# csyxwei/FFWM

Measured on AMD Instinct MI355X. Metric: train img/s (128x128, full FFWM GAN step), higher is better.
Workload: dtype f32; 1 GPU; BASELINE configs[2]: full FFWM train step (netG+netD+flowNetF+flowNetB, all losses, 3x Adam), synthetic MultiPIE-shaped 128x128; batch_per_gpu=8, global_batch=8, parallelism=dp1, grad_buckets=10, bucket_MiB=64

## Files before the change

### ffwm_amd/_lib.py

```python
import ctypes
import os

_HERE = os.path.dirname(os.path.abspath(__file__))
LIB_PATH = os.path.join(_HERE, "lib", "libffwm_hip.so")

F32, F64 = 0, 1
ABI_VERSION = 5

_lib = None

_p = ctypes.c_void_p
_i64 = ctypes.c_int64
_i = ctypes.c_int

_SIGNATURES = {
    "ffwm_block_extractor_forward": [_p, _p, _p] + [_i64] * 6 + [_i, _i, _p],
    "ffwm_block_extractor_backward": [_p, _p, _p, _p, _p] + [_i64] * 6 + [_i, _i, _p],
    "ffwm_block_extractor_backward_strided": [_p, _p, _p, ctypes.POINTER(_i64), _p, _p] + [_i64] * 6 + [_i, _i, _p],
    "ffwm_local_attn_reshape_backward_strided": [_p, ctypes.POINTER(_i64), _p] + [_i64] * 3 + [_i, _i, _i, _p],
    "ffwm_resample2d_backward_strided": [_p, _p, _p, ctypes.POINTER(_i64), _p, _p] + [_i64] * 6 + [_i, _i, _i, _i, _p],
    "ffwm_bn_lrelu_forward": [_p] * 9 + [_i64] * 3 + [ctypes.c_double] * 3 + [_i, _p],
    "ffwm_bn_lrelu_backward": [_p] * 10 + [_i64] * 3 + [ctypes.c_double] + [_i, _p],
    "ffwm_bn_res_act_forward": [_p] * 11 + [_i64] * 3 + [ctypes.c_double] * 3 + [_i, _i, _p],
    "ffwm_bn_res_act_backward": [_p] * 11 + [_i64] * 3 + [ctypes.c_double] + [_i, _i, _p],
# ... 3 lines not shown
    "ffwm_add_act_backward": [_p, _p, _p, _i64, _i, ctypes.c_double, _i, _p],
    "ffwm_sigmoid_gate_forward": [_p, _p, _p, _p, _p, _i64, _i, _p],
    "ffwm_sigmoid_gate_backward": [_p, _p, _p, _p, _p, _i64, _i, _p],
    "ffwm_bias_relu_forward": [_p, _p, _p] + [_i64] * 3 + [_i, _p],
    "ffwm_bias_act_forward": [_p, _p, _p, _p] + [_i64] * 5 + [_i, ctypes.c_double, _i, _p],
    "ffwm_flow_head_forward": [_p, _p, _p, _p] + [_i64] * 4 + [_i, _p],
    "ffwm_conv_thin_forward": [_p, _p, _p, _p] + [_i64] * 5 + [_i, ctypes.c_double, _i, _p],
    "ffwm_flow_up_forward": [_p, _p, _p, _p] + [_i64] * 4 + [_i, _p],
    "ffwm_shuffle_bias_act_forward": [_p, _p, _p] + [_i64] * 5 + [ctypes.c_double, _i, _p],
    "ffwm_image_head_forward": [_p, _p, _p, _p] + [_i64] * 5 + [_i, _p],
    "ffwm_upsample2x_bilinear_forward": [_p, _p] + [_i64] * 5 + [_i, _p],
    "ffwm_sigmoid_gate_forward_strided": [_p, _p, _p, _p, _p] + [_i64] * 4 + [_i, _p],
    "ffwm_flow_head_backward": [_p, _p, _p, _p, _p] + [_i64] * 4 + [_i, _p],
    "ffwm_flow_up_backward": [_p, _p, _p] + [_i64] * 4 + [_i, _p],
    "ffwm_conv2d_forward": [_p, _p, _p, _p, _p] + [_i64] * 5 + [_i, _i, _i, _i, _i64, _i64, _i, ctypes.c_double, _p, _i64, _i, _p],
    "ffwm_conv2d_wgrad": [_p, _p, _p] + [_i64] * 7 + [_i, _i, _i, _i, _p],
    "ffwm_conv2d_wgrad_tiled": [_p, _p, _p, _p] + [_i64] * 7 + [_i, _i, _i, _i, _i, _p],
    "ffwm_conv3x3_winograd_forward": [_p, _p, _p, _p, _p] + [_i64] * 5 + [_i, _i, ctypes.c_double, _i, _p],
    "ffwm_adam_step": [_p, _p, _p, _p, _i64] + [ctypes.c_double] * 4 + [_i64, _i, _p],
    "ffwm_adam_step_device": [_p, _p, _p, _p, _i64] + [ctypes.c_double] * 4 + [_p, _i, _p],
    "ffwm_sgd_step": [_p, _p, _p, _i64, _p, _p, _i, _p, _p, _i, ctypes.c_double, _i, _p],
    "ffwm_softmax_xent": [_p] * 8 + [_i64, _i64, _i, _p],
    "ffwm_softmax_xent_chunk": [],
    "ffwm_conv3x3_wgrad": [_p, _p, _p, _p] + [_i64] * 5 + [_i, _p],
    "ffwm_conv3x3_wgrad_block": [_p, _p, _p, _p] + [_i64] * 9 + [_i, _p],
    "ffwm_block_attention_forward": [_p, _p, _p, _p] + [_i64] * 6 + [_i, _i, _p],
    "ffwm_block_attention_backward": [_p, _p, _p, _p, _p, _p, _p] + [_i64] * 6 + [_i, _i, _p],
    "ffwm_local_attn_reshape_forward": [_p, _p] + [_i64] * 3 + [_i, _i, _p],
    "ffwm_local_attn_reshape_backward": [_p, _p] + [_i64] * 3 + [_i, _i, _i, _p],
    "ffwm_resample2d_forward": [_p, _p, _p] + [_i64] * 6 + [_i, _i, _i, _p],
    "ffwm_resample2d_backward": [_p, _p, _p, _p, _p] + [_i64] * 6 + [_i, _i, _i, _i, _p],
    "ffwm_warp_forward": [_p, _p, _p] + [_i64] * 6 + [_i, _i, _p],
    "ffwm_warp_backward": [_p, _p, _p, _p, _p] + [_i64] * 6 + [_i, _i, _p],
    "ffwm_warp_multi_forward": [_p, _i, _i, _i, _p],
    "ffwm_warp_multi_backward": [_p, _i, _i, _i, _p],
    "ffwm_spectral_norm_forward": [_p, _i, _i, ctypes.c_double, _i, _p],
    "ffwm_spectral_norm_backward": [_p, _i, _i, _p],
    "ffwm_guided_filter_forward": [_p, _p, _p, _p, _i64, _i64, _i64, _i, ctypes.c_double, _i, _p],
    "ffwm_affine_regularization": [_p, _p, _p, _p, _i64, _i64, _i64, _i, ctypes.c_double, _i, _p],
    "ffwm_correlation_colmax": [_p, _p, _p, _i64, _i64, _i64, _i, _p],
    "ffwm_correlation_colmax_split": [_p, _p, _p, _i64, _i64, _i64, _i, _p],
    "ffwm_sampling_correctness": [_p] * 9 + [_i64] * 6 + [ctypes.c_double, ctypes.c_double, _i, _p],
    "ffwm_landmark_loss": [_p, _p, ctypes.POINTER(_i64), ctypes.POINTER(_i64), ctypes.POINTER(ctypes.c_double), _i] + [_p] * 6
                          + [_i64, _i64, _i, _p],
    "ffwm_guided_filter_backward": [_p, _p, _p, _p, _p, _p, _i64, _i64, _i64, _i, _i, _p],
    "ffwm_guided_filter_forward_general": [_p, _p, _p, _p, _p, _i64, _i64, _i64, _i64, _i, ctypes.c_double, _i, _p],
    "ffwm_guided_filter_backward_general": [_p, _p, _p, _p, _p, _p, _p, _i64, _i64, _i64, _i64, _i, _i, _p],
    "ffwm_l1_multi": [_p, _i, _p, _p, _i, _i, _p],
    "ffwm_conv3x3_winograd_weights_multi": [_p, _i, _i, _p],
    "ffwm_conv3x3_wg_weights": [_p, _p, _i64, _i64, _i, _i, _p],
    "ffwm_conv3x3_wg_forward": [_p, _p, _p, _p, _p] + [_i64] * 5 + [_i, _p, _i, _p],
    "ffwm_conv3x3_wg_forward_tiled": [_p, _p, _p, _p, _p] + [_i64] * 5 + [_i, _p, _i, _i, _p],
    "ffwm_conv3x3_wg_tile": [_i64] * 5,
    "ffwm_mfm_tail_forward": [_p, _p, _p, _p] + [_i64] * 4 + [_i, _i, _p],
    "ffwm_identity_input": [_p, _p] + [_i64] * 4 + [_i, _i, _p],
    "ffwm_identity_input_backward": [_p, _p] + [_i64] * 4 + [_i, _i, _p],
    "ffwm_cosine_topk": [_p, _p, _p, _p] + [_i64] * 4 + [_p, _i64, _i, _p],
    "ffwm_prof_enable": [_i],
    "ffwm_prof_collect": [],
    "ffwm_prof_get": [_i, ctypes.c_char_p, _i, ctypes.POINTER(_i64), ctypes.POINTER(ctypes.c_double),
                      ctypes.POINTER(ctypes.c_double)],
    "ffwm_prof_get_flops": [_i, ctypes.POINTER(ctypes.c_double)],
    "ffwm_prof_get_bound": [_i, ctypes.POINTER(ctypes.c_double)],
    "ffwm_prof_reset": [],
    "ffwm_set_option": [ctypes.c_char_p, _i],
    "ffwm_zero_fill": [_p, _i64, _p],
    "ffwm_abi_version": [],
}

EXPORTS = sorted(list(_SIGNATURES) + ["ffwm_last_error", "ffwm_conv3x3_winograd_workspace_bytes", "ffwm_conv3x3_winograd_splits",
                                      "ffwm_conv2d_forward_workspace", "ffwm_guided_filter_workspace_bytes",
                                      "ffwm_sampling_correctness_workspace_bytes", "ffwm_landmark_loss_workspace_bytes",
                                      "ffwm_cosine_topk_workspace_bytes", "ffwm_softmax_xent_workspace_bytes",
                                      "ffwm_conv3x3_wg_weights_bytes", "ffwm_conv3x3_wg_workspace_bytes"])


class FFWMError(RuntimeError):
    pass


def load():
    global _lib
    if _lib is not None:
        return _lib
    if not os.path.exists(LIB_PATH):
        raise FFWMError(
            "libffwm_hip.so is missing (%s). The HIP extension is the only implementation of the "
            "ffwm_amd ops -- build it with `python -m ffwm_amd.build`." % LIB_PATH)
    lib = ctypes.CDLL(LIB_PATH)
    for name, argtypes in _SIGNATURES.items():
        fn = getattr(lib, name)
        fn.argtypes = argtypes
        fn.restype = _i
    lib.ffwm_conv3x3_winograd_workspace_bytes.argtypes = [_i64, _i64]
    lib.ffwm_conv3x3_winograd_workspace_bytes.restype = _i64
    lib.ffwm_conv3x3_winograd_splits.argtypes = [_i64, _i64, _i64, _i64, _i64, _i]
    lib.ffwm_conv3x3_winograd_splits.restype = _i
    lib.ffwm_conv2d_forward_workspace.argtypes = [_i64] * 5 + [_i] * 4
    lib.ffwm_conv2d_forward_workspace.restype = _i64
    lib.ffwm_guided_filter_workspace_bytes.argtypes = [_i64] * 4 + [_i, _i]
    lib.ffwm_guided_filter_workspace_bytes.restype = _i64
    lib.ffwm_sampling_correctness_workspace_bytes.argtypes = [_i64, _i64, _i64, _i]
    lib.ffwm_sampling_correctness_workspace_bytes.restype = _i64
    lib.ffwm_landmark_loss_workspace_bytes.argtypes = [ctypes.POINTER(_i64), _i, _i64, _i64, _i]
    lib.ffwm_landmark_loss_workspace_bytes.restype = _i64
    lib.ffwm_softmax_xent_workspace_bytes.argtypes = [_i64, _i64, _i]
# ... 62 lines not shown
```

### ffwm_amd/conv.py

```python
import os as _os

import torch
import torch.nn as nn
from torch.autograd import Function

from . import ops

_WGRAD_W64 = _os.environ.get("FFWM_WGRAD_W64", "1") == "1"


class _Conv3x3MfmaWgrad(Function):

    @staticmethod
    def forward(ctx, x, weight, bias):
        ctx.save_for_backward(x, weight)
        ctx.has_bias = bias is not None
        return torch.ops.aten.convolution(x, weight, bias, [1, 1], [1, 1], [1, 1], False, [0, 0], 1)

    @staticmethod
    @torch.autograd.function.once_differentiable
    def backward(ctx, grad_output):
        x, weight = ctx.saved_tensors
        go = grad_output.contiguous()
        need_x, need_w, need_b = ctx.needs_input_grad[0], ctx.needs_input_grad[1], ctx.has_bias and ctx.needs_input_grad[2]
# ... 373 lines not shown
        if ctx.own_dgrad:
            return ops.conv3x3_wg(go, ctx.entry[1], None, "none", relu_mask=y, K=ctx.C), None, None, None, None
        if ctx.relu:
            go = torch.ops.aten.threshold_backward(go, y, 0)
        gx = torch.ops.aten.convolution_backward(go, x, weight, None, [1, 1], [1, 1], [1, 1], False, [0, 0], 1, [True, False, False])[0]
        return gx, None, None, None, None


def wg_bias_relu(x, layer):
    entry = wg_entry(layer, layer.weight)
    if torch.is_grad_enabled() and x.requires_grad:
        return _WgConv3x3.apply(x, layer.weight, layer.bias, entry, True)
    return ops.conv3x3_wg(x.contiguous(), entry[0], layer.bias, "relu")


def wg_conv(x, layer):
    entry = wg_entry(layer, layer.weight)
    if torch.is_grad_enabled() and x.requires_grad:
        return _WgConv3x3.apply(x, layer.weight, None, entry, False)
    return ops.conv3x3_wg(x.contiguous(), entry[0], None, "none", K=layer.weight.shape[0])


def wg_bias_mfm(x, layer):
    entry = wg_entry(layer, layer.weight)
    return ops.conv3x3_wg(x.contiguous(), entry[0], layer.bias, "mfm", K=layer.weight.shape[0])


def wg_prepare(net):
    n = 0
    if not _WG:
        return n
    for m in net.modules():
        if (isinstance(m, nn.Conv2d) and m.kernel_size == (3, 3) and m.stride == (1, 1) and m.padding == (1, 1) and m.dilation == (1, 1)
                and m.groups == 1 and m.weight.is_cuda and m.weight.dtype == torch.float32 and _wg_class(m.weight)[0] != _WG_NEVER):
            d = wg_entry(m, m.weight)
            if d is not None:
                n += 4 * sum(u.numel() for k, u in d.items() if k != "key")
    return n


def _conv_fwd_call(x, weight, bias, stride, pad, transposed):
    from .flownet_eval import conv_mfma, NONE
    return conv_mfma(x, weight, bias, stride, pad, transposed, NONE)


def _bias_grad(go):
    return go.sum((0, 2, 3))


_OWN_DGRAD = _os.environ.get("FFWM_CONV_DGRAD", "0") == "1"
_OWN_DGRAD_T = _os.environ.get("FFWM_CONVT_DGRAD", "1") != "0"


class _MfmaConv2d(Function):

    @staticmethod
    def forward(ctx, x, weight, bias, stride, pad, own_fwd=True):
        x, weight = x.contiguous(), weight.contiguous()
        ctx.save_for_backward(x, weight)
        ctx.cfg = (stride, pad, bias is not None)
        if own_fwd:
            return _conv_fwd_call(x, weight, bias, stride, pad, False)
        return torch.ops.aten.convolution(x, weight, bias, [stride, stride], [pad, pad], [1, 1], False, [0, 0], 1)

    @staticmethod
    @torch.autograd.function.once_differentiable
    def backward(ctx, grad_output):
        x, weight = ctx.saved_tensors
        stride, pad, has_bias = ctx.cfg
        go = grad_output.contiguous()
        need_x, need_w, need_b = ctx.needs_input_grad[0], ctx.needs_input_grad[1], has_bias and ctx.needs_input_grad[2]
        gx = gw = gb = None
        k = weight.size(2)
        even = x.size(2) == 2 * go.size(2) and x.size(3) == 2 * go.size(3)
        if need_x and _OWN_DGRAD and stride == 2 and pad == 1 and even and min(weight.shape[0], weight.shape[1]) >= 32:
            gx = _conv_fwd_call(go, weight, None, 2, 1, 1 if k == 4 else 2)
            need_x = False
        elif (need_x and k == 3 and stride == 1 and pad == 1 and min(weight.shape[0], weight.shape[1]) >= 32
              and (_OWN_DGRAD or x.size(2) * x.size(3) <= 64)):
            gx = _conv_fwd_call(go, weight, None, 1, 1, 3)
            need_x = False
        if need_w:
            gw, gb = conv_weight_grad(x, go, weight, stride, pad, need_b)
        if need_x:
            gx = torch.ops.aten.convolution_backward(go, x, weight, None, [stride, stride], [pad, pad], [1, 1], False, [0, 0], 1,
                                                     [True, False, False])[0]
        if need_b and gb is None:
            gb = _bias_grad(go)
        return gx, gw, gb, None, None, None


class _MfmaConvTranspose2d(Function):

    @staticmethod
    def forward(ctx, x, weight, bias, own_fwd=True):
        x, weight = x.contiguous(), weight.contiguous()
        ctx.save_for_backward(x, weight)
        ctx.has_bias = bias is not None
        if own_fwd:
            return _conv_fwd_call(x, weight, bias, 2, 1, True)
        return torch.ops.aten.convolution(x, weight, bias, [2, 2], [1, 1], [1, 1], True, [0, 0], 1)

    @staticmethod
    @torch.autograd.function.once_differentiable
    def backward(ctx, grad_output):
        x, weight = ctx.saved_tensors
        go = grad_output.contiguous()
        need_x, need_w, need_b = ctx.needs_input_grad[0], ctx.needs_input_grad[1], ctx.has_bias and ctx.needs_input_grad[2]
        gx = gw = gb = None
        if need_x and _OWN_DGRAD_T and min(weight.shape[0], weight.shape[1]) >= 16:
            gx = _conv_fwd_call(go, weight, None, 2, 1, False)
            need_x = False
        if need_w:
            gw, gb = conv_transpose_weight_grad(x, go, weight, need_b)
        if need_x:
            gx = torch.ops.aten.convolution_backward(go, x, weight, None, [2, 2], [1, 1], [1, 1], True, [0, 0], 1, [True, False, False])[0]
        if need_b and gb is None:
            gb = _bias_grad(go)
        return gx, gw, gb, None


def fwd_route_ok(x, weight):
    return (x.is_cuda and x.dtype == torch.float32 and weight.dtype == torch.float32 and x.dim() == 4 and not torch.is_autocast_enabled()
            and x.numel() < (1 << 29) and weight.numel() < (1 << 29))


class MfmaFwdConv2d(nn.Conv2d):

    def _conv_forward(self, input, weight, bias):
        if fwd_route_ok(input, weight) and (self.stride[0] == 2 or input.size(2) <= 32):
            return _MfmaConv2d.apply(input, weight, bias, self.stride[0], self.padding[0])
        return super()._conv_forward(input, weight, bias)

# ... 192 lines not shown
```

### ffwm_amd/nets.py

```python
import math
import os

import torch
import torch.nn as nn
import torch.nn.functional as F
from torch.nn.utils import spectral_norm

from . import _ext
from . import conv as _conv
from .external_function import WarpFlipCat, WarpNet, warp_many

LRELU = 0.2


def _msra(mods):
    for m in mods:
        if isinstance(m, (nn.Conv2d, nn.ConvTranspose2d)):
            nn.init.kaiming_normal_(m.weight)
            if m.bias is not None:
                nn.init.constant_(m.bias, 0)


def _cbl(cin, cout, stride=1):
    return nn.Sequential(nn.Conv2d(cin, cout, 3, stride, 1, bias=True), nn.BatchNorm2d(cout),
# ... 45 lines not shown
        f = self.conv0(x)
        skips = {}
        for L in range(1, 7):
            f = getattr(self, "conv%d_1" % L)(getattr(self, "conv%d" % L)(f))
            skips[L] = f
        flow = self.predict_flow6(f)
        flows = {}
        cat = None
        for L in range(5, -1, -1):
            up = getattr(self, "upsampled_flow%d_to_%d" % (L + 1, L))(flow)
            d = getattr(self, "deconv%d" % L)(f if L == 5 else cat)
            cat = torch.cat((skips[L], d, up) if L >= 3 else (d, up), 1)
            flow = getattr(self, "predict_flow%d" % L)(getattr(self, "inter_conv%d" % L)(cat))
            flows[L] = flow
        return flows[0], flows[1], flows[2]


class Tanh2(nn.Module):
    def forward(self, x):
        return (torch.tanh(x) + 1) / 2


def _activ(name):
    table = {"relu": nn.ReLU, "lrelu": lambda: nn.LeakyReLU(LRELU), "sigmoid": nn.Sigmoid, "tanh": nn.Tanh,
             "tanh2": Tanh2}
    if name not in table:
        raise NotImplementedError("Activation %s not implemented" % name)
    return table[name]()


def _sn(m, on):
    return spectral_norm(m) if on else m


class ResidualBlock(nn.Module):

    def __init__(self, inc, outc=None, kernel=3, activ="lrelu", sn=True):
        super().__init__()
        outc = inc if outc is None else outc
        pad = kernel // 2 if sn else kernel
        self.activ = _activ(activ)
        self.input = _sn(nn.Conv2d(inc, outc, 1, 1, 0), sn)
        self.blocks = nn.Sequential(_sn(nn.Conv2d(inc, outc, kernel, 1, pad), sn), nn.BatchNorm2d(outc),
                                    nn.LeakyReLU(LRELU), _sn(nn.Conv2d(outc, outc, kernel, 1, pad), sn),
                                    nn.BatchNorm2d(outc))

    def forward(self, x):
        return self.activ(self.blocks(x) + self.input(x))


class FusedResidualBlock(ResidualBlock):

    def forward(self, x):
        from .norm import RES_ACTS, bn_res_act, bn_res_act_ok
        from .residual import _act_of, add_act
        blocks, inp = self.blocks, self.input
        bn = blocks[-1] if isinstance(blocks, nn.Sequential) and len(blocks) >= 2 else None
        act, slope = _act_of(self.activ)
        if (bn is not None and isinstance(inp, nn.Conv2d) and not inp._forward_pre_hooks and not inp._forward_hooks
                and bn_res_act_ok(bn, x, RES_ACTS.get(act)) and torch.is_grad_enabled()):
            h = x
            for m in list(blocks)[:-1]:
                h = m(h)
            s = inp._conv_forward(x, inp.weight, None)
            if h.shape == s.shape and h.shape[1] == bn.num_features:
                return bn_res_act(h, bn, s, inp.bias, RES_ACTS[act], slope)
            return add_act(bn(h), s if inp.bias is None else s + inp.bias.view(1, -1, 1, 1), self.activ)
        return add_act(blocks(x), inp(x), self.activ)


def _conv_block(inc, outc, ks, s, p, activ="lrelu", res=0, bn=True, sn=True):
    layers = [_sn(nn.Conv2d(inc, outc, ks, s, p), sn)]
    if bn:
        layers.append(nn.BatchNorm2d(outc))
    if activ is not None:
        layers.append(_activ(activ))
    layers += [ResidualBlock(outc, activ=activ, sn=sn) for _ in range(res)]
    return nn.Sequential(*layers)


def _shuffle_block(inc, outc, sn=True):
    return nn.Sequential(_sn(nn.Conv2d(inc, outc * 4, 3, 1, 1), sn), nn.PixelShuffle(2), nn.BatchNorm2d(outc),
                         _activ("lrelu"))


class FFWM(nn.Module):

    def __init__(self, num_layers=3, isflip=True, sn=True, warp_flipcat=None):
        super().__init__()
        ch = [64, 64, 128, 256]
        dch = [256, 128, 64, 64]
        self.isflip = isflip
        dm = 3 if isflip else 2
        am = dm - 1
        self.layers = num_layers
        self.e0 = _conv_block(3, ch[0], 7, 1, 3, res=1, bn=False, sn=sn)
        for i in (1, 2, 3):
            setattr(self, "e%d" % i, _conv_block(ch[i - 1], ch[i], 4, 2, 1, res=1, sn=sn))
        d_in = [dch[0], dch[1] * dm, dch[2] * dm + 3]
        r_ch = [dch[1] * dm, dch[2] * dm + 3, dch[3] * dm + 3]
        for i in range(3):
            setattr(self, "d%d" % i, _shuffle_block(d_in[i], dch[i + 1], sn=sn))
        for i in range(3):
            setattr(self, "dres%d" % i, nn.Sequential(*[ResidualBlock(r_ch[i], activ="lrelu", sn=sn) for _ in range(2)]))
        for i in range(3):
            setattr(self, "rec%d" % i, _conv_block(r_ch[i], 3, 3, 1, 1, bn=False, activ="sigmoid", sn=sn))
        for i, c in enumerate((ch[2] * am, ch[1] * am, ch[0] * am)):
            setattr(self, "att%d" % i, nn.Sequential(_conv_block(c, c, 3, 1, 1, sn=sn),
                                                     ResidualBlock(c, c, activ="sigmoid", sn=sn)))
        self.warpNet = WarpNet()
        self._fused = warp_flipcat if warp_flipcat is not None else WarpFlipCat()
        self._multi = warp_flipcat is None and os.environ.get("FFWM_WARP_MULTI", "1") != "0"
        self.fuse_gate = False

    def _skip(self, feat, flow):
        if self.isflip:
            return self._fused(feat, flow)
# ... 263 lines not shown
```

### ffwm_amd/ops.py

```python
import ctypes

import torch

from . import _lib

_DT = {torch.float32: _lib.F32, torch.float64: _lib.F64}


def _dtype_code(t):
    try:
        return _DT[t.dtype]
    except KeyError:
        raise TypeError("ffwm_amd ops support float32/float64 (AT_DISPATCH_FLOATING_TYPES), got %s" % t.dtype)


def _go_strides(grad_output):
    if grad_output.is_contiguous():
        return grad_output, None
    st = grad_output.stride()
    if any(x < 0 for x in st) or st[3] == 0:
        return grad_output.contiguous(), None
    return grad_output, (ctypes.c_int64 * 4)(*st)


# ... 739 lines not shown

WG_EPILOGUES = {"none": 0, "bias": 1, "relu": 2, "mfm": 3}


def conv3x3_wg_weights(weight, data_gradient=False):
    if not (weight.is_cuda and weight.dtype == torch.float32 and weight.is_contiguous() and weight.dim() == 4 and tuple(weight.shape[2:]) == (3, 3)):
        raise ValueError("conv3x3_wg_weights: a contiguous float32 [K, C, 3, 3] weight on the GPU")
    K, C = (weight.shape[1], weight.shape[0]) if data_gradient else (weight.shape[0], weight.shape[1])
    lib = _lib.load()
    U = weight.new_empty((lib.ffwm_conv3x3_wg_weights_bytes(K, C) // 4,))
    with _on_device(weight) as stream:
        _lib.check(lib.ffwm_conv3x3_wg_weights(_ptr(weight), _ptr(U), K, C, int(bool(data_gradient)), _lib.F32, stream), "ffwm_conv3x3_wg_weights")
    return U


def conv3x3_wg(x, U, bias, epilogue, relu_mask=None, out=None, K=None, tile=0):
    _check("conv3x3_wg", x, relu_mask, out)
    for t in (U, bias):
        if t is not None and (t.device != x.device or t.dtype != x.dtype or not t.is_contiguous()):
            raise ValueError("conv3x3_wg: U and bias must be contiguous tensors of the input's device and dtype")
    if x.dtype != torch.float32:
        raise TypeError("conv3x3_wg: float32 only")
    B, C, H, W = x.shape
    if K is None:
        if bias is None:
            raise ValueError("conv3x3_wg: K is needed when there is no bias")
        K = bias.numel()
    lib = _lib.load()
    if U.numel() * 4 != lib.ffwm_conv3x3_wg_weights_bytes(K, C):
        raise ValueError("conv3x3_wg: U does not belong to a layer with %d input and %d output channels" % (C, K))
    if bias is not None and (not bias.is_contiguous() or bias.numel() != K):
        raise ValueError("conv3x3_wg: bias must be a contiguous vector of %d elements" % K)
    if relu_mask is not None and (relu_mask.shape != x.shape or not relu_mask.is_contiguous()):
        raise ValueError("conv3x3_wg: relu_mask must be contiguous and of x's shape")
    epi = WG_EPILOGUES[epilogue]
    if epi == 3 and K % 2:
        raise ValueError("conv3x3_wg: the mfm epilogue needs an even K")
    shape = (B, K // 2 if epi == 3 else K, H, W)
    if out is None:
        out = x.new_empty(shape)
    elif tuple(out.shape) != shape:
        raise ValueError("conv3x3_wg: out has the wrong shape")
    ws = x.new_empty((lib.ffwm_conv3x3_wg_workspace_bytes(B, C, H, W, K) // 4,))
    with _on_device(x) as stream:
        _lib.check(lib.ffwm_conv3x3_wg_forward_tiled(_ptr(x), _ptr(U), _ptr(bias), _ptr(out), _ptr(ws), B, C, H, W, K, epi,
                                                     _ptr(relu_mask), int(tile), _dtype_code(x), stream), "ffwm_conv3x3_wg_forward")
    return out


def conv3x3_wg_tile(B, C, H, W, K):
    return int(_lib.load().ffwm_conv3x3_wg_tile(int(B), int(C), int(H), int(W), int(K)))


def _mfm_dims(x):
    if x.dim() < 2 or x.shape[1] % 2:
        raise ValueError("mfm: need [B, 2C, ...], got %s" % (tuple(x.shape),))
    hw = 1
    for d in x.shape[2:]:
        hw *= d
    return x.shape[0], x.shape[1] // 2, hw


def _bias_ok(x, bias, n):
    if bias is None:
        return
    if not (bias.is_cuda and bias.dtype == x.dtype and bias.is_contiguous() and bias.numel() == n):
        raise ValueError("bias must be a contiguous float32 GPU vector of %d elements" % n)


_ACT_CODES = {"lrelu": 1, "sigmoid": 3}


def _same_f32(name, *ts):
    t0 = ts[0]
    for t in ts:
        if not (t.is_cuda and t.dtype == torch.float32 and t.is_contiguous() and t.shape == t0.shape and t.device == t0.device):
            raise NotImplementedError("%s: contiguous float32 GPU tensors of one shape only" % name)


def add_act_forward(a, b, act, negative_slope=0.2):
    _same_f32("add_act_forward", a, b)
    y = torch.empty_like(a)
    if y.numel():
        with _on_device(a) as stream:
            _lib.check(_lib.load().ffwm_add_act_forward(_ptr(a), _ptr(b), _ptr(y), a.numel(), _ACT_CODES[act], float(negative_slope),
                                                        _lib.F32, stream), "ffwm_add_act_forward")
    return y


def add_act_backward(y, grad_y, act, negative_slope=0.2):
    _same_f32("add_act_backward", y, grad_y)
    dz = torch.empty_like(y)
    if dz.numel():
        with _on_device(y) as stream:
            _lib.check(_lib.load().ffwm_add_act_backward(_ptr(y), _ptr(grad_y), _ptr(dz), y.numel(), _ACT_CODES[act],
                                                         float(negative_slope), _lib.F32, stream), "ffwm_add_act_backward")
    return dz


def sigmoid_gate_forward(a, b, x):
    _same_f32("sigmoid_gate_forward", a, b, x)
    att, y = torch.empty_like(a), torch.empty_like(a)
    if y.numel():
        with _on_device(a) as stream:
            _lib.check(_lib.load().ffwm_sigmoid_gate_forward(_ptr(a), _ptr(b), _ptr(x), _ptr(att), _ptr(y), a.numel(), _lib.F32, stream),
                       "ffwm_sigmoid_gate_forward")
# ... 257 lines not shown
```

### ffwm_amd/residual.py

```python
import torch
import torch.nn as nn
from torch.autograd import Function
from torch.autograd.function import once_differentiable

from . import ops


class _AddAct(Function):
    @staticmethod
    def forward(ctx, a, b, act, slope):
        y = ops.add_act_forward(a.contiguous(), b.contiguous(), act, slope)
        ctx.save_for_backward(y)
        ctx.act, ctx.slope = act, slope
        return y

    @staticmethod
    @once_differentiable
    def backward(ctx, g):
        (y,) = ctx.saved_tensors
        dz = ops.add_act_backward(y, _grad_in(g), ctx.act, ctx.slope)
        return dz, dz, None, None


class _SigmoidGate(Function):
    @staticmethod
    def forward(ctx, a, b, x):
        x = x.contiguous()
        y, att = ops.sigmoid_gate_forward(a.contiguous(), b.contiguous(), x)
        ctx.save_for_backward(x, att)
        ctx.mark_non_differentiable(att)
        return y, att

    @staticmethod
    @once_differentiable
    def backward(ctx, gy, _gatt):
        x, att = ctx.saved_tensors
        dz, dx = ops.sigmoid_gate_backward(x, att, _grad_in(gy))
        return dz, dz, dx


def _act_of(module):
    if isinstance(module, nn.LeakyReLU) and module.negative_slope > 0:
        return "lrelu", float(module.negative_slope)
    if isinstance(module, nn.Sigmoid):
        return "sigmoid", 0.0
    return None, 0.0


def _aligned(t):
    return not t.is_contiguous() or t.data_ptr() % 16 == 0


def _kernel_ok(*ts):
    t0 = ts[0]
    return (t0.is_cuda and not torch.is_autocast_enabled()
            and all(t.dtype == torch.float32 and t.shape == t0.shape and t.device == t0.device and _aligned(t) for t in ts))


def _grad_in(g):
    g = g.contiguous()
    return g if g.data_ptr() % 16 == 0 else g.clone()


def add_act(a, b, activ):
    act, slope = _act_of(activ)
    if act is not None and _kernel_ok(a, b):
        return _AddAct.apply(a, b, act, slope)
    return activ(a + b)


def gated(att_module, skip, fuse=True):
    rb = att_module[-1] if isinstance(att_module, nn.Sequential) and len(att_module) >= 2 else None
    if (fuse and rb is not None and hasattr(rb, "blocks") and hasattr(rb, "input") and isinstance(getattr(rb, "activ", None), nn.Sigmoid)
            and _kernel_ok(skip)):
        h = skip
        for m in list(att_module)[:-1]:
            h = m(h)
        a, b = rb.blocks(h), rb.input(h)
        if _kernel_ok(a, b, skip):
            return _SigmoidGate.apply(a, b, skip)
        att = rb.activ(a + b)
        return skip * att, att
    att = att_module(skip)
    return skip * att, att


def fuse_residual(net):
    from .nets import FusedResidualBlock, ResidualBlock
    n = 0
    for m in net.modules():
        if type(m) is ResidualBlock and _act_of(m.activ)[0] is not None:
            m.__class__ = FusedResidualBlock
            n += 1
    if hasattr(net, "fuse_gate"):
        net.fuse_gate = True
    return n
```

### include/ffwm_hip.h

```cpp
#ifndef FFWM_HIP_H_
#define FFWM_HIP_H_

#include <stdint.h>

#ifdef __cplusplus
extern "C" {
#endif

#define FFWM_ABI_VERSION 5

typedef enum {
    FFWM_OK = 0,
    FFWM_ERR_ARG = -1,
    FFWM_ERR_DTYPE = -2,
    FFWM_ERR_SIZE = -3,
    FFWM_ERR_LAUNCH = -4
} ffwm_status;

typedef enum { FFWM_F32 = 0, FFWM_F64 = 1 } ffwm_dtype;

int ffwm_abi_version(void);
const char* ffwm_last_error(void);

int ffwm_block_extractor_forward(const void* source, const void* flow_field, void* output,
// ... 187 lines not shown
                           int64_t K, int act, double negative_slope, int dtype, void* stream);

int ffwm_flow_head_forward(const void* x, const void* weight, const void* bias, void* y, int64_t B, int64_t C, int64_t H,
                           int64_t W, int dtype, void* stream);
int ffwm_flow_up_forward(const void* flow, const void* weight, const void* bias, void* out, int64_t B, int64_t H, int64_t W,
                         int64_t out_batch_stride, int dtype, void* stream);

int ffwm_flow_head_backward(const void* y, const void* grad_y, const void* weight, void* grad_z, void* grad_x, int64_t B, int64_t C,
                            int64_t H, int64_t W, int dtype, void* stream);
int ffwm_flow_up_backward(const void* grad_out, const void* weight, void* grad_x, int64_t B, int64_t H, int64_t W,
                          int64_t grad_out_batch_stride, int dtype, void* stream);

int64_t ffwm_conv2d_forward_workspace(int64_t B, int64_t C, int64_t H, int64_t W, int64_t K, int kernel, int stride, int pad,
                                      int transposed);
int ffwm_conv2d_forward(const void* input, const void* weight, const void* bias, void* output, void* output2, int64_t B, int64_t C,
                        int64_t H, int64_t W, int64_t K, int kernel, int stride, int pad, int transposed, int64_t out_batch_stride,
                        int64_t out2_batch_stride, int act, double negative_slope, void* workspace, int64_t workspace_bytes,
                        int dtype, void* stream);

int ffwm_conv2d_wgrad(const void* rows, const void* gathered, void* grad_weight, int64_t B, int64_t K, int64_t Ho, int64_t Wo,
                      int64_t C, int64_t H, int64_t W, int kernel, int stride, int pad, int dtype, void* stream);

int ffwm_conv2d_wgrad_tiled(const void* rows, const void* gathered, void* grad_weight, void* grad_bias, int64_t B, int64_t K,
                            int64_t Ho, int64_t Wo, int64_t C, int64_t H, int64_t W, int kernel, int stride, int pad, int prezeroed,
                            int dtype, void* stream);

int64_t ffwm_conv3x3_winograd_workspace_bytes(int64_t K, int64_t C);
int ffwm_conv3x3_winograd_splits(int64_t B, int64_t C, int64_t H, int64_t W, int64_t K, int act);

typedef struct ffwm_wino_weights {
    const void* weight;
    void* workspace;
    int64_t K, C;
    int data_gradient;
    int width_multiple_of_4;
} ffwm_wino_weights;
int ffwm_conv3x3_winograd_weights_multi(const ffwm_wino_weights* items, int n, int dtype, void* stream);
int ffwm_conv3x3_winograd_forward(const void* input, const void* weight, const void* bias, void* output, void* workspace,
                                  int64_t B, int64_t C, int64_t H, int64_t W, int64_t K, int data_gradient, int act,
                                  double slope, int dtype, void* stream);

enum { FFWM_WG_NONE = 0, FFWM_WG_BIAS = 1, FFWM_WG_BIAS_RELU = 2, FFWM_WG_BIAS_MFM = 3 };
int64_t ffwm_conv3x3_wg_weights_bytes(int64_t K, int64_t C);
int64_t ffwm_conv3x3_wg_workspace_bytes(int64_t B, int64_t C, int64_t H, int64_t W, int64_t K);
int ffwm_conv3x3_wg_weights(const void* weight, void* U, int64_t K, int64_t C, int data_gradient, int dtype, void* stream);
int ffwm_conv3x3_wg_forward(const void* input, const void* U, const void* bias, void* output, void* workspace,
                            int64_t B, int64_t C, int64_t H, int64_t W, int64_t K, int epilogue, const void* relu_mask,
                            int dtype, void* stream);
int ffwm_conv3x3_wg_tile(int64_t B, int64_t C, int64_t H, int64_t W, int64_t K);
int ffwm_conv3x3_wg_forward_tiled(const void* input, const void* U, const void* bias, void* output, void* workspace,
                                  int64_t B, int64_t C, int64_t H, int64_t W, int64_t K, int epilogue, const void* relu_mask,
                                  int tile, int dtype, void* stream);

int ffwm_adam_step(void* params, const void* grads, void* exp_avg, void* exp_avg_sq, int64_t n, double lr,
                   double beta1, double beta2, double eps, int64_t step, int dtype, void* stream);

int ffwm_adam_step_device(void* params, const void* grads, void* exp_avg, void* exp_avg_sq, int64_t n, double lr, double beta1,
                          double beta2, double eps, void* state, int dtype, void* stream);

int ffwm_sgd_step(void* params, const void* grads, void* momentum_buf, int64_t n, const int64_t* seg_end, const int32_t* seg_group,
                  int n_seg, const double* group_lr, const double* group_wd, int n_groups, double momentum, int dtype, void* stream);

int ffwm_softmax_xent_chunk(void);
int64_t ffwm_softmax_xent_workspace_bytes(int64_t B, int64_t N, int dtype);
int ffwm_softmax_xent(const void* logits, const int64_t* target, void* out, void* row_loss, int* rank, void* grad_logits,
                      int* skipped, void* workspace, int64_t B, int64_t N, int dtype, void* stream);

int ffwm_shuffle_bias_act_forward(const void* h, const void* bias, void* y, int64_t B, int64_t K, int64_t H, int64_t W,
                                  int64_t y_batch_stride, double negative_slope, int dtype, void* stream);
int ffwm_image_head_forward(const void* x, const void* weight, const void* bias, void* y, int64_t B, int64_t C, int64_t H, int64_t W,
                            int64_t y_batch_stride, int dtype, void* stream);
int ffwm_upsample2x_bilinear_forward(const void* x, void* y, int64_t B, int64_t C, int64_t H, int64_t W, int64_t y_batch_stride,
                                     int dtype, void* stream);
int ffwm_sigmoid_gate_forward_strided(const void* a, const void* b, const void* x, void* att, void* y, int64_t B, int64_t C,
                                      int64_t HW, int64_t y_batch_stride, int dtype, void* stream);

int ffwm_mfm_tail_forward(const void* h, const void* bias, const void* residual, void* y, int64_t B, int64_t C, int64_t H, int64_t W,
                          int pool, int dtype, void* stream);
int ffwm_identity_input(const void* img, void* out, int64_t B, int64_t Cin, int64_t H, int64_t W, int crop, int dtype, void* stream);
int ffwm_identity_input_backward(const void* grad_out, void* grad_img, int64_t B, int64_t Cin, int64_t H, int64_t W, int crop, int dtype,
                                 void* stream);
int64_t ffwm_cosine_topk_workspace_bytes(int64_t B, int64_t G, int64_t D, int64_t k);
int ffwm_cosine_topk(const void* probe, const void* gallery, void* values, void* indices, int64_t B, int64_t G, int64_t D, int64_t k,
                     void* workspace, int64_t workspace_bytes, int dtype, void* stream);

int ffwm_prof_enable(int on);
int ffwm_prof_collect(void);
int ffwm_prof_get(int row, char* name, int name_len, int64_t* launches, double* total_ms,
                  double* algorithmic_bytes);
int ffwm_prof_get_flops(int row, double* algorithmic_flops);
int ffwm_prof_get_bound(int row, double* roofline_ms);
int ffwm_prof_reset(void);

int ffwm_set_option(const char* key, int value);

int ffwm_zero_fill(void* p, int64_t bytes, void* stream);

#ifdef __cplusplus
}
#endif
#endif
```

Baseline: 219.9 img/s.

## Add MFMA 1x1 conv kernel with fused residual dgrad for shortcut convs

Adds a HIP kernel for 1x1 convolutions that uses fp32 MFMA (32x32x2) with double-buffered LDS weight staging and an optional residual add in the epilogue. A shape/pixel-count table decides per layer whether forward and data-gradient go through this kernel or through aten. A new autograd function forks the residual-block shortcut so the shortcut-conv data gradient is fused with the main-branch gradient accumulation, saving a separate add. The aim is to reduce the cost of library 1x1 convs and gradient sums, at the price of a hand-tuned table and more custom-kernel code.

```diff
diff --git a/ffwm_amd/_lib.py b/ffwm_amd/_lib.py
--- a/ffwm_amd/_lib.py
+++ b/ffwm_amd/_lib.py
@@ -79,6 +79,7 @@
     "ffwm_conv3x3_wg_forward": [_p, _p, _p, _p, _p] + [_i64] * 5 + [_i, _p, _i, _p],
     "ffwm_conv3x3_wg_forward_tiled": [_p, _p, _p, _p, _p] + [_i64] * 5 + [_i, _p, _i, _i, _p],
     "ffwm_conv3x3_wg_tile": [_i64] * 5,
+    "ffwm_conv1x1_forward": [_p, _p, _p, _p] + [_i64] * 5 + [_i, _i, _p],
     "ffwm_mfm_tail_forward": [_p, _p, _p, _p] + [_i64] * 4 + [_i, _i, _p],
     "ffwm_identity_input": [_p, _p] + [_i64] * 4 + [_i, _i, _p],
     "ffwm_identity_input_backward": [_p, _p] + [_i64] * 4 + [_i, _i, _p],
diff --git a/ffwm_amd/conv.py b/ffwm_amd/conv.py
--- a/ffwm_amd/conv.py
+++ b/ffwm_amd/conv.py
@@ -449,6 +449,82 @@
 _OWN_DGRAD_T = _os.environ.get("FFWM_CONVT_DGRAD", "1") != "0"
 
 
+_CONV1X1 = _os.environ.get("FFWM_CONV1X1", "1") != "0"
+_C1_NEVER = (1, 0)
+CONV1X1_TABLE = {
+    (64, 64): ((32768, 131072), (32768, 131072)),
+    (128, 128): ((32768, 32768), (8192, 131072)),
+    (195, 195): ((32768, 131072), (32768, 131072)),
+    (256, 256): (_C1_NEVER, (2048, 2048)),
+    (384, 384): (_C1_NEVER, _C1_NEVER),
+}
+CONV1X1_UNLISTED = (_C1_NEVER, _C1_NEVER)
+
+
+def _conv1x1_layer_ok(x, weight):
+    return (_CONV1X1 and weight.dim() == 4 and weight.shape[2] == 1 and weight.shape[3] == 1 and x.dim() == 4
+            and weight.shape[1] == x.shape[1] and min(weight.shape[0], weight.shape[1]) >= 32 and not torch.is_autocast_enabled()
+            and ops.conv1x1_ok(x, weight))
+
+
+def conv1x1_dirs(x, weight):
+    if not _conv1x1_layer_ok(x, weight):
+        return False, False
+    pixels = x.shape[0] * x.shape[2] * x.shape[3]
+    fwd, dgrad = CONV1X1_TABLE.get((weight.shape[1], weight.shape[0]), CONV1X1_UNLISTED)
+    return fwd[0] <= pixels <= fwd[1], dgrad[0] <= pixels <= dgrad[1]
+
+
+def _conv1x1_dgrad(go, x, weight, own, join=None):
+    if own and ops.conv1x1_ok(go, weight, join):
+        return ops.conv1x1(go, weight, transposed=True, residual=join)
+    gx = torch.ops.aten.convolution_backward(go, x, weight, None, [1, 1], [0, 0], [1, 1], False, [0, 0], 1, [True, False, False])[0]
+    return gx if join is None else join + gx
+
+
+class _ShortcutFork(Function):
+
+    @staticmethod
+    def forward(ctx, x, weight, bias, dirs):
+        ctx.set_materialize_grads(False)
+        ctx.save_for_backward(x, weight)
+        ctx.has_bias, ctx.own_dgrad = bias is not None, dirs[1]
+        if dirs[0]:
+            s = ops.conv1x1(x, weight)
+            if bias is not None:
+                s += bias.view(1, -1, 1, 1)
+        else:
+            s = torch.ops.aten.convolution(x, weight, bias, [1, 1], [0, 0], [1, 1], False, [0, 0], 1)
+        return x, s
+
+    @staticmethod
+    @torch.autograd.function.once_differentiable
+    def backward(ctx, g_main, g_s):
+        x, weight = ctx.saved_tensors
+        need_x, need_w, need_b = ctx.needs_input_grad[0], ctx.needs_input_grad[1], ctx.has_bias and ctx.needs_input_grad[2]
+        if g_s is None:
+            return (g_main if need_x else None), None, None, None
+        go = g_s.contiguous()
+        gx = gw = gb = None
+        if need_x:
+            gx = _conv1x1_dgrad(go, x, weight, ctx.own_dgrad, None if g_main is None else g_main.contiguous())
+        if need_w:
+            gw, gb = conv_weight_grad(x, go, weight, 1, 0, need_b)
+        if need_b and gb is None:
+            gb = _bias_grad(go)
+        return gx, gw, gb, None
+
+
+def shortcut_fork(layer, x, with_bias):
+    if (type(layer) is OwnBwdConv2d and layer.kernel_size == (1, 1) and layer.stride == (1, 1) and layer.padding == (0, 0)
+            and not layer._forward_pre_hooks and not layer._forward_hooks
+            and torch.is_grad_enabled() and layer.weight.requires_grad and x.requires_grad and x.is_contiguous()):
+        dirs = conv1x1_dirs(x, layer.weight)
+        if dirs[0] or dirs[1]:
+            return _ShortcutFork.apply(x, layer.weight, layer.bias if with_bias else None, dirs)
+    return x, (layer(x) if with_bias else layer._conv_forward(x, layer.weight, None))
+
+
 class _MfmaConv2d(Function):
 
     @staticmethod
@@ -456,8 +532,14 @@
         x, weight = x.contiguous(), weight.contiguous()
         ctx.save_for_backward(x, weight)
         ctx.cfg = (stride, pad, bias is not None)
+        ctx.c1 = conv1x1_dirs(x, weight) if (not own_fwd and stride == 1 and pad == 0) else (False, False)
         if own_fwd:
             return _conv_fwd_call(x, weight, bias, stride, pad, False)
+        if ctx.c1[0]:
+            y = ops.conv1x1(x, weight)
+            if bias is not None:
+                y += bias.view(1, -1, 1, 1)
+            return y
         return torch.ops.aten.convolution(x, weight, bias, [stride, stride], [pad, pad], [1, 1], False, [0, 0], 1)
 
     @staticmethod
@@ -476,6 +558,9 @@
         elif (need_x and k == 3 and stride == 1 and pad == 1 and min(weight.shape[0], weight.shape[1]) >= 32
               and (_OWN_DGRAD or x.size(2) * x.size(3) <= 64)):
             gx = _conv_fwd_call(go, weight, None, 1, 1, 3)
+            need_x = False
+        elif need_x and ctx.c1[1]:
+            gx = _conv1x1_dgrad(go, x, weight, True)
             need_x = False
         if need_w:
             gw, gb = conv_weight_grad(x, go, weight, stride, pad, need_b)
diff --git a/ffwm_amd/csrc/conv1x1.hip b/ffwm_amd/csrc/conv1x1.hip
--- /dev/null
+++ b/ffwm_amd/csrc/conv1x1.hip
@@ -0,0 +1,210 @@
+#include "common.hpp"
+
+namespace ffwm {
+namespace {
+
+typedef float f32x16 __attribute__((ext_vector_type(16)));
+
+constexpr int kC1Stage = 16;
+constexpr int kC1MaxRB = 8;
+
+constexpr unsigned kC1Nowhere = 0x80000000u;
+
+template <int CB>
+struct C1Vec {
+    union {
+        float v[CB];
+        unsigned w[CB];
+    };
+};
+
+__device__ __forceinline__ unsigned c1_nowhere_if_negative(int v) { return static_cast<unsigned>(v) & kC1Nowhere; }
+
+template <int RB, int CB, int TR>
+__global__ void __launch_bounds__(kBlock, 2)
+conv1x1_kernel(const float* __restrict__ x, const float* __restrict__ w, const float* res, float* out, int C, int K, int P,
+               unsigned total, int groups) {
+    constexpr int ROWS = RB * 32, LD = ROWS + 1, NA = kC1Stage * ROWS / kBlock, NS = kC1Stage / 2;
+    __shared__ float Ws[2][kC1Stage][LD];
+    const int lane = threadIdx.x & 63, wave = threadIdx.x >> 6;
+    const int l31 = lane & 31, half = lane >> 5;
+    const unsigned lb = xcd_remap(blockIdx.x, gridDim.x, 1);
+    const int grp = static_cast<int>(lb % static_cast<unsigned>(groups));
+    const unsigned strip = lb / static_cast<unsigned>(groups);
+    const int k0 = grp * ROWS;
+
+    const rsrc_t xr = make_rsrc(x, static_cast<unsigned>(total) * static_cast<unsigned>(C) * 4u);
+    const rsrc_t wr = make_rsrc(w, static_cast<unsigned>(K) * static_cast<unsigned>(C) * 4u);
+    const rsrc_t orr = make_rsrc(out, static_cast<unsigned>(total) * static_cast<unsigned>(K) * 4u);
+    const rsrc_t rr = make_rsrc(res != nullptr ? res : out, static_cast<unsigned>(total) * static_cast<unsigned>(K) * 4u);
+
+    const unsigned pix = (strip * 4u + wave) * (32u * CB) + CB * l31;
+    const bool pv = pix < total;
+    const unsigned b = pv ? pix / static_cast<unsigned>(P) : 0u;
+    const unsigned p = pv ? pix - b * static_cast<unsigned>(P) : 0u;
+    const unsigned P4 = static_cast<unsigned>(P) * 4u;
+    const unsigned xoff = pv ? (b * static_cast<unsigned>(C)) * P4 + p * 4u : kC1Nowhere;
+
+    auto wload = [&](int st, float (&ra)[NA]) {
+#pragma unroll
+        for (int n = 0; n < NA; ++n) {
+            const int e = threadIdx.x + kBlock * n;
+            const int c = TR ? e / ROWS : e & (kC1Stage - 1);
+            const int k = TR ? e % ROWS : e >> 4;
+            const int cg = st * kC1Stage + c, kg = k0 + k;
+            const unsigned o = static_cast<unsigned>(TR ? cg * K + kg : kg * C + cg) * 4u;
+            ra[n] = buf_ld<float>(wr, o | c1_nowhere_if_negative((C - 1 - cg) | (K - 1 - kg)));
+        }
+    };
+    auto wstore = [&](int buf, const float (&ra)[NA]) {
+#pragma unroll
+        for (int n = 0; n < NA; ++n) {
+            const int e = threadIdx.x + kBlock * n;
+            const int c = TR ? e / ROWS : e & (kC1Stage - 1);
+            const int k = TR ? e % ROWS : e >> 4;
+            Ws[buf][c][k] = ra[n];
+        }
+    };
+    auto bload = [&](int st, C1Vec<CB> (&rb)[NS]) {
+#pragma unroll
+        for (int s = 0; s < NS; ++s) {
+            const int c = st * kC1Stage + 2 * s + half;
+            buf_load_dwords<CB>(xr, (xoff + static_cast<unsigned>(c) * P4) | c1_nowhere_if_negative(C - 1 - c), rb[s].w);
+        }
+    };
+
+    f32x16 acc[RB][CB];
+#pragma unroll
+    for (int i = 0; i < RB; ++i)
+#pragma unroll
+        for (int j = 0; j < CB; ++j)
+#pragma unroll
+            for (int r = 0; r < 16; ++r) acc[i][j][r] = 0.f;
+
+    float ra[NA];
+    C1Vec<CB> rb[NS], bc[NS];
+    const int stages = (C + kC1Stage - 1) / kC1Stage;
+    wload(0, ra);
+    bload(0, rb);
+    wstore(0, ra);
+    __syncthreads();
+    int buf = 0;
+    for (int st = 0; st < stages; ++st) {
+        const bool more = st + 1 < stages;
+#pragma unroll
+        for (int s = 0; s < NS; ++s) bc[s] = rb[s];
+        if (more) {
+            wload(st + 1, ra);
+            bload(st + 1, rb);
+        }
+        float a[2][RB];
+#pragma unroll
+        for (int i = 0; i < RB; ++i) a[0][i] = Ws[buf][half][i * 32 + l31];
+#pragma unroll
+        for (int s = 0; s < NS; ++s) {
+            if (s + 1 < NS) {
+#pragma unroll
+                for (int i = 0; i < RB; ++i) a[(s + 1) & 1][i] = Ws[buf][2 * (s + 1) + half][i * 32 + l31];
+            }
+#pragma unroll
+            for (int i = 0; i < RB; ++i)
+#pragma unroll
+                for (int j = 0; j < CB; ++j) acc[i][j] = __builtin_amdgcn_mfma_f32_32x32x2f32(a[s & 1][i], bc[s].v[j], acc[i][j], 0, 0, 0);
+        }
+        if (more) wstore(buf ^ 1, ra);
+        __syncthreads();
+        buf ^= 1;
+    }
+
+    const unsigned obase = pv ? (b * static_cast<unsigned>(K)) * P4 + p * 4u : kC1Nowhere;
+#pragma unroll
+    for (int i = 0; i < RB; ++i) {
+        unsigned off[16];
+        C1Vec<CB> q[16];
+#pragma unroll
+        for (int r = 0; r < 16; ++r) {
+            const int row = k0 + i * 32 + (r & 3) + 8 * (r >> 2) + 4 * half;
+            off[r] = (obase + static_cast<unsigned>(row) * P4) | c1_nowhere_if_negative(K - 1 - row);
+        }
+        if (res != nullptr) {
+#pragma unroll
+            for (int r = 0; r < 16; ++r) buf_load_dwords<CB>(rr, off[r], q[r].w);
+        }
+#pragma unroll
+        for (int r = 0; r < 16; ++r) {
+            C1Vec<CB> v;
+#pragma unroll
+            for (int j = 0; j < CB; ++j) v.v[j] = res != nullptr ? q[r].v[j] + acc[i][j][r] : acc[i][j][r];
+            buf_store_dwords<CB>(orr, off[r], v.w);
+        }
+    }
+}
+
+}
+}
+
+using namespace ffwm;
+
+struct C1Plan {
+    int RB, CB;
+    int64_t groups, strips;
+};
+static C1Plan c1_plan(int64_t total, int64_t K) {
+    const int64_t cus = device_cus();
+    const int64_t rbt = (K + 31) / 32;
+    const int64_t gmin = (rbt + kC1MaxRB - 1) / kC1MaxRB;
+    C1Plan p;
+    auto cut = [&](int cb) {
+        p.CB = cb;
+        p.strips = (total + 128 * cb - 1) / (128 * cb);
+        int64_t g = (cus + p.strips - 1) / p.strips;
+        if (g > rbt) g = rbt;
+        if (g < gmin) g = gmin;
+        p.RB = static_cast<int>((rbt + g - 1) / g);
+        p.groups = (rbt + p.RB - 1) / p.RB;
+    };
+    cut(2);
+    if (p.RB > 4 || p.strips * p.groups < cus) cut(1);
+    return p;
+}
+
+extern "C" int ffwm_conv1x1_forward(const void* input, const void* weight, const void* residual, void* output, int64_t B, int64_t C,
+                                    int64_t H, int64_t W, int64_t K, int transposed, int dtype, void* stream) {
+    const char* fn = "ffwm_conv1x1_forward";
+    FFWM_REQUIRE(dtype == FFWM_F32, FFWM_ERR_DTYPE, "%s: float32 only", fn);
+    FFWM_REQUIRE(input && weight && output, FFWM_ERR_ARG, "%s: NULL tensor pointer", fn);
+    FFWM_REQUIRE(B > 0 && C > 0 && H > 0 && W > 0 && K > 0, FFWM_ERR_ARG, "%s: sizes must be positive", fn);
+    FFWM_REQUIRE(transposed == 0 || transposed == 1, FFWM_ERR_ARG, "%s: transposed must be 0 or 1", fn);
+    FFWM_REQUIRE(H < (1LL << 31) / W, FFWM_ERR_SIZE, "%s: a plane beyond 2^31 elements", fn);
+    const int64_t P = H * W;
+    FFWM_REQUIRE(P % 4 == 0, FFWM_ERR_ARG, "%s: H W must be a multiple of 4", fn);
+    FFWM_REQUIRE(reinterpret_cast<uintptr_t>(input) % 16 == 0 && reinterpret_cast<uintptr_t>(output) % 16 == 0 &&
+                     reinterpret_cast<uintptr_t>(residual) % 16 == 0,
+                 FFWM_ERR_ARG, "%s: input, residual and output must be 16-byte aligned", fn);
+    FFWM_REQUIRE(B < (1LL << 29) / P && C < (1LL << 29) / (B * P) && K < (1LL << 29) / (B * P) && K * C < (1LL << 29), FFWM_ERR_SIZE,
+                 "%s: a tensor of 2^29 elements or more", fn);
+    const int64_t total = B * P;
+    const C1Plan p = c1_plan(total, K);
+    FFWM_REQUIRE(p.strips * p.groups < (1LL << 31) && p.strips * 128 * p.CB < (1LL << 32), FFWM_ERR_SIZE, "%s: too many workgroups", fn);
+    hipStream_t st = static_cast<hipStream_t>(stream);
+    LaunchScope ls("conv1x1", st, 4.0 * (static_cast<double>(total) * C + static_cast<double>(K) * C +
+                                         static_cast<double>(total) * K * (residual ? 2.0 : 1.0)),
+                   2.0 * static_cast<double>(total) * K * C);
+    const bool ok = dispatch<1, 2, 3, 4, 5, 6, 7, 8>(p.RB, [&](auto RB) {
+        return dispatch<1, 2>(p.CB, [&](auto CB) {
+            return dispatch<0, 1>(transposed, [&](auto TR) {
+                if constexpr (CB.value == 2 && (RB.value > 4)) {
+                    return false;
+                } else {
+                    hipLaunchKernelGGL((conv1x1_kernel<RB.value, CB.value, TR.value>), dim3(static_cast<unsigned>(p.strips * p.groups)),
+                                       dim3(kBlock), 0, st, static_cast<const float*>(input), static_cast<const float*>(weight),
+                                       static_cast<const float*>(residual), static_cast<float*>(output), static_cast<int>(C),
+                                       static_cast<int>(K), static_cast<int>(P), static_cast<unsigned>(total), static_cast<int>(p.groups));
+                    return true;
+                }
+            });
+        });
+    });
+    if (!ok) return no_kernel(fn);
+    return check_launch(fn);
+}
diff --git a/ffwm_amd/nets.py b/ffwm_amd/nets.py
--- a/ffwm_amd/nets.py
+++ b/ffwm_amd/nets.py
@@ -121,6 +121,7 @@
 class FusedResidualBlock(ResidualBlock):
 
     def forward(self, x):
+        from .conv import shortcut_fork
         from .norm import RES_ACTS, bn_res_act, bn_res_act_ok
         from .residual import _act_of, add_act
         blocks, inp = self.blocks, self.input
@@ -128,10 +129,9 @@
         act, slope = _act_of(self.activ)
         if (bn is not None and isinstance(inp, nn.Conv2d) and not inp._forward_pre_hooks and not inp._forward_hooks
                 and bn_res_act_ok(bn, x, RES_ACTS.get(act)) and torch.is_grad_enabled()):
-            h = x
+            h, s = shortcut_fork(inp, x, False)
             for m in list(blocks)[:-1]:
                 h = m(h)
-            s = inp._conv_forward(x, inp.weight, None)
             if h.shape == s.shape and h.shape[1] == bn.num_features:
                 return bn_res_act(h, bn, s, inp.bias, RES_ACTS[act], slope)
             return add_act(bn(h), s if inp.bias is None else s + inp.bias.view(1, -1, 1, 1), self.activ)
diff --git a/ffwm_amd/ops.py b/ffwm_amd/ops.py
--- a/ffwm_amd/ops.py
+++ b/ffwm_amd/ops.py
@@ -815,6 +815,39 @@
     return int(_lib.load().ffwm_conv3x3_wg_tile(int(B), int(C), int(H), int(W), int(K)))
 
 
+def conv1x1_ok(x, weight, residual=None):
+    if not (x.is_cuda and x.dtype == torch.float32 and x.dim() == 4 and x.is_contiguous() and x.data_ptr() % 16 == 0
+            and (x.shape[2] * x.shape[3]) % 4 == 0 and 0 < x.numel() < (1 << 29)):
+        return False
+    if not (weight.is_cuda and weight.device == x.device and weight.dtype == torch.float32 and weight.is_contiguous()
+            and weight.dim() in (2, 4) and weight.numel() == weight.shape[0] * weight.shape[1] and weight.numel() < (1 << 29)):
+        return False
+    if residual is not None and not (residual.is_cuda and residual.device == x.device and residual.dtype == torch.float32
+                                     and residual.is_contiguous() and residual.data_ptr() % 16 == 0):
+        return False
+    return True
+
+
+def conv1x1(x, weight, transposed=False, residual=None, out=None):
+    _check("conv1x1", x, residual, out)
+    if not conv1x1_ok(x, weight, residual):
+        raise ValueError("conv1x1: contiguous 16-byte aligned float32 GPU tensors, H W a multiple of 4, a contiguous [K, C(, 1, 1)] weight")
+    B, C, H, W = x.shape
+    K = weight.shape[1] if transposed else weight.shape[0]
+    if (weight.shape[0] if transposed else weight.shape[1]) != C:
+        raise ValueError("conv1x1: weight %s does not match %d input channels" % (tuple(weight.shape), C))
+    shape = (B, K, H, W)
+    if out is None:
+        out = x.new_empty(shape)
+    for t in (out, residual):
+        if t is not None and (tuple(t.shape) != shape or t.data_ptr() % 16 or t.numel() >= (1 << 29)):
+            raise ValueError("conv1x1: out / residual must be 16-byte aligned [B, K, H, W] tensors")
+    with _on_device(x) as stream:
+        _lib.check(_lib.load().ffwm_conv1x1_forward(_ptr(x), _ptr(weight), _ptr(residual), _ptr(out), B, C, H, W, K,
+                                                    1 if transposed else 0, _lib.F32, stream), "ffwm_conv1x1_forward")
+    return out
+
+
 def _mfm_dims(x):
     if x.dim() < 2 or x.shape[1] % 2:
         raise ValueError("mfm: need [B, 2C, ...], got %s" % (tuple(x.shape),))
diff --git a/ffwm_amd/residual.py b/ffwm_amd/residual.py
--- a/ffwm_amd/residual.py
+++ b/ffwm_amd/residual.py
@@ -76,7 +76,9 @@
         h = skip
         for m in list(att_module)[:-1]:
             h = m(h)
-        a, b = rb.blocks(h), rb.input(h)
+        from .conv import shortcut_fork
+        hm, b = shortcut_fork(rb.input, h, True)
+        a = rb.blocks(hm)
         if _kernel_ok(a, b, skip):
             return _SigmoidGate.apply(a, b, skip)
         att = rb.activ(a + b)
diff --git a/include/ffwm_hip.h b/include/ffwm_hip.h
--- a/include/ffwm_hip.h
+++ b/include/ffwm_hip.h
@@ -263,6 +263,9 @@
                                   int64_t B, int64_t C, int64_t H, int64_t W, int64_t K, int epilogue, const void* relu_mask,
                                   int tile, int dtype, void* stream);
 
+int ffwm_conv1x1_forward(const void* input, const void* weight, const void* residual, void* output, int64_t B, int64_t C, int64_t H,
+                         int64_t W, int64_t K, int transposed, int dtype, void* stream);
+
 int ffwm_adam_step(void* params, const void* grads, void* exp_avg, void* exp_avg_sq, int64_t n, double lr,
                    double beta1, double beta2, double eps, int64_t step, int dtype, void* stream);
 
```

Result: no change. 220.2 img/s (median of 3 runs) (+0.1%).
